# Tangshitao/Semi-supervised-Adaptive-Distillation

Measured on AMD Instinct MI355X. Metric: images/sec (student+teacher fwd + student bwd) R50-FPN distill, 1/2/4/8 MI355X, higher is better.
Workload: dtype f32

## Files before the change

### include/ssad_kernels.h

```cpp
#ifndef SSAD_KERNELS_H_
#define SSAD_KERNELS_H_

#include <stddef.h>
#include <stdint.h>

#ifdef __cplusplus
extern "C" {
#endif

#define SSAD_API __attribute__((visibility("default")))

#define SSAD_E_BADARG (-1)
#define SSAD_E_WORKSPACE (-2)
#define SSAD_MAX_LEVELS 8
#define SSAD_MAX_CONV_PROBLEMS 24
#define SSAD_MAX_POWSUM_INPUTS 8

typedef void* ssad_stream_t;


typedef struct {
  float gamma;
  float alpha;
  float beta;
// ... 176 lines not shown
    const float* bias, int Cout, int Cin, int flags, ssad_stream_t stream);

SSAD_API size_t ssad_conv_split_filter_floats(int M, int K);
SSAD_API int ssad_conv_split_pack_filters(const ssad_pack_entry* entries_host, int n_entries, ssad_stream_t stream);
SSAD_API size_t ssad_conv3x3_split_workspace_bytes(const ssad_conv_level* levels_host, int n_levels, int Cin);
SSAD_API int ssad_conv3x3_forward_split(
    const ssad_conv_level* levels_host, int n_levels, const float* packed,
    const float* bias, int Cout, int Cin, int flags, void* workspace, size_t workspace_bytes,
    const unsigned* amax_in, unsigned* amax_out, ssad_stream_t stream);

SSAD_API size_t ssad_conv3x3_wgrad_workspace_bytes(
    const ssad_conv_level* levels_host, int n_levels, int Cout, int Cin);

SSAD_API int ssad_conv3x3_wgrad(
    const ssad_conv_level* levels_host, int n_levels, float* dW, float* db,
    int Cout, int Cin, int accumulate, void* workspace, size_t workspace_bytes,
    ssad_stream_t stream);

SSAD_API size_t ssad_conv3x3_wgrad_split_workspace_bytes(
    const ssad_conv_level* levels_host, int n_levels, int Cout, int Cin);
SSAD_API int ssad_conv3x3_wgrad_split(
    const ssad_conv_level* levels_host, int n_levels, float* dW, float* db,
    int Cout, int Cin, int accumulate, void* workspace, size_t workspace_bytes,
    ssad_stream_t stream);
SSAD_API int ssad_conv3x3_wgrad_split_amax(
    const ssad_conv_level* levels_host, int n_levels, float* dW, float* db,
    int Cout, int Cin, int accumulate, void* workspace, size_t workspace_bytes,
    const unsigned* x_amax, const unsigned* dy_amax, ssad_stream_t stream);

SSAD_API int ssad_split_absmax_levels(const ssad_conv_level* levels_host, int n, int channels, int field,
                                      unsigned* words, ssad_stream_t stream);
SSAD_API int ssad_split_absmax(const float* x, long long n, unsigned* word, ssad_stream_t stream);


SSAD_API size_t ssad_retinanet_anchor_labels_workspace_bytes(
    int levels, int A, int k_min, const int* field_sizes_host, int N, int Gmax);
SSAD_API int ssad_retinanet_anchor_labels(
    const double* cell_anchors, int levels, int A, int k_min, const int* field_sizes_host,
    const int* crop_h_host, const int* crop_w_host, const float* gt_boxes,
    const int* gt_classes, const int* gt_counts, int N, int Gmax, int num_classes,
    float positive_overlap, float negative_overlap, int* const* labels_out_host,
    float* const* locs_out_host, float* const* targets_out_host, int capacity,
    int* counts_out, float* fg_bg_out, void* workspace, size_t workspace_bytes,
    ssad_stream_t stream);


SSAD_API int ssad_conv_out_size(int in, int kernel, int dilation, int pad_a, int pad_b, int stride);
SSAD_API int ssad_im2col(const float* x, int C, int H, int W, int kh, int kw, int dil_h, int dil_w,
                         int pad_t, int pad_l, int pad_b, int pad_r, int stride_h, int stride_w,
                         float* col, ssad_stream_t stream);
SSAD_API int ssad_im2col_batched(const float* x, int N, int C, int H, int W, int kernel, int stride,
                                 int pad, float* col, ssad_stream_t stream);
SSAD_API int ssad_col2im(const float* col, int C, int H, int W, int kh, int kw, int dil_h,
                         int dil_w, int pad_t, int pad_l, int pad_b, int pad_r, int stride_h,
                         int stride_w, float* x, ssad_stream_t stream);
SSAD_API int ssad_channel_sum(const float* dy, int N, int C, int HW, float* out, int accumulate,
                              ssad_stream_t stream);
SSAD_API int ssad_relu_grad_rowsum(const float* y, const float* dy, float* dx, float* rowsum, int N,
                                   int C, int HW, ssad_stream_t stream);
SSAD_API int ssad_conv1x1_bias_act(const float* x, const float* w, const float* bias,
                                   const float* residual, float* y, int N, int C, int P, int M,
                                   int relu, ssad_stream_t stream);
SSAD_API int ssad_conv1x1_bias_act2(const float* x, int C1, const float* x2, int C2, const float* w,
                                    const float* bias, const float* residual, float* y, int N, int P,
                                    int M, int relu, ssad_stream_t stream);
#define SSAD_GEMM_RELU 1
#define SSAD_GEMM_ACCUMULATE 8
typedef struct ssad_gemm_conv {
  const float* a;
  const float* x;
  float* y;
  const float* bias;
  const float* residual;
  const float* mask;
  int lda, N, K, P, M, flags;
} ssad_gemm_conv;
SSAD_API int ssad_conv1x1_gemm(const ssad_gemm_conv* desc_host, ssad_stream_t stream);
SSAD_API size_t ssad_conv1x1_gemm_split_workspace_bytes(const ssad_gemm_conv* desc_host);
SSAD_API int ssad_conv1x1_gemm_split(const ssad_gemm_conv* desc_host, void* workspace, size_t workspace_bytes,
                                     ssad_stream_t stream);
SSAD_API int ssad_conv1x1_gemm_split_amax(const ssad_gemm_conv* desc_host, const float* packed_a, const unsigned* x_amax,
                                          unsigned* y_amax_out, void* workspace, size_t workspace_bytes,
                                          ssad_stream_t stream);
typedef struct ssad_gemm_pack_entry {
  const float* a;
  float* dst;
  int lda, K, M;
} ssad_gemm_pack_entry;
SSAD_API size_t ssad_gemm_split_filter_floats(int K, int M);
SSAD_API int ssad_gemm_split_pack_filters(const ssad_gemm_pack_entry* entries_host, int n_entries, ssad_stream_t stream);
SSAD_API int ssad_conv_implicit_gemm(const ssad_gemm_conv* d, int C, int H, int W, int kernel, int stride, int pad,
                                     ssad_stream_t stream);
SSAD_API size_t ssad_conv_implicit_gemm_workspace_bytes(int N, int M, int C, int H, int W, int kernel, int stride,
                                                        int pad);
SSAD_API int ssad_conv_implicit_gemm_ws(const ssad_gemm_conv* d, int C, int H, int W, int kernel, int stride, int pad,
                                        void* workspace, size_t workspace_bytes, ssad_stream_t stream);
SSAD_API size_t ssad_conv_kxk_wgrad_workspace_bytes(int N, int C, int H, int W, int M, int kernel, int stride,
                                                    int pad);
SSAD_API int ssad_conv_kxk_wgrad(const float* x, const float* dy, int N, int C, int H, int W, int M, int kernel,
                                 int stride, int pad, float* dw, int accumulate, void* workspace,
                                 size_t workspace_bytes, ssad_stream_t stream);
SSAD_API size_t ssad_conv_kxk_dgrad_workspace_bytes(int N, int C, int H, int W, int M, int kernel, int stride,
                                                    int pad);
SSAD_API int ssad_conv_kxk_dgrad(const float* w, const float* dy, int N, int C, int H, int W, int M, int kernel,
                                 int stride, int pad, float* dx, const float* mask, int accumulate, void* workspace,
                                 size_t workspace_bytes, ssad_stream_t stream);
SSAD_API int ssad_transpose_filter(const float* w, int M, int K, int ldm, float* wt, ssad_stream_t stream);
#define SSAD_MAX_TRANSPOSE_ENTRIES 64
typedef struct ssad_transpose_entry {
  const float* w;
  float* wt;
  int M, K, ldm;
  int reserved;
} ssad_transpose_entry;
SSAD_API int ssad_transpose_filters(const ssad_transpose_entry* entries_host, int n_entries, ssad_stream_t stream);
SSAD_API size_t ssad_conv1x1_wgrad_workspace_bytes(int N, int C, int P, int M);
SSAD_API int ssad_conv1x1_wgrad(const float* x, const float* dy, int N, int C, int P, int M, float* dw,
                                int accumulate, void* workspace, size_t workspace_bytes,
                                ssad_stream_t stream);
SSAD_API size_t ssad_conv1x1_wgrad_split_workspace_bytes(int N, int C, int P, int M);
SSAD_API int ssad_conv1x1_wgrad_split(const float* x, const float* dy, int N, int C, int P, int M, float* dw,
                                      int accumulate, void* workspace, size_t workspace_bytes,
                                      ssad_stream_t stream);
SSAD_API int ssad_conv1x1_wgrad_split_amax(const float* x, const float* dy, int N, int C, int P, int M, float* dw,
                                           int accumulate, void* workspace, size_t workspace_bytes,
                                           const unsigned* x_amax, const unsigned* dy_amax, ssad_stream_t stream);
SSAD_API int ssad_subsample(const float* x, int N, int C, int H, int W, int stride, float* y,
                            ssad_stream_t stream);
SSAD_API int ssad_subsample_grad(const float* dy, int N, int C, int H, int W, int stride, int accumulate,
                                 float* dx, ssad_stream_t stream);
SSAD_API long long ssad_grouped_conv3x3_filter_floats(int C, int group);
SSAD_API int ssad_grouped_conv3x3_pack_filter(const float* w, int C, int group, float* packed,
                                              ssad_stream_t stream);
SSAD_API int ssad_grouped_conv3x3_forward(const float* x, const float* packed, const float* bias, int N, int C,
                                          int H, int W, int group, int stride, int relu, float* y,
                                          ssad_stream_t stream);
SSAD_API int ssad_max_pool_forward(const float* x, int N, int C, int H, int W, int kh, int kw,
                                   int stride_h, int stride_w, int pad_t, int pad_l, int pad_b,
                                   int pad_r, float* y, ssad_stream_t stream);
SSAD_API int ssad_max_pool3x3s2_bias_relu(const float* x, const float* bias, int N, int C, int H,
                                          int W, int relu, float* y, ssad_stream_t stream);
SSAD_API int ssad_max_pool_backward(const float* x, const float* y, const float* dy, int N, int C,
                                    int H, int W, int kh, int kw, int stride_h, int stride_w,
                                    int pad_t, int pad_l, int pad_b, int pad_r, float* dx,
                                    ssad_stream_t stream);

SSAD_API size_t ssad_retinanet_detect_workspace_bytes(
    int levels, int A, int C, const int* H_host, const int* W_host, int pre_nms_topn);
SSAD_API int ssad_retinanet_detect(
    const float* const* cls_prob_host, const float* const* box_pred_host,
    const double* cell_anchors, int levels, int A, int C, int k_min, const int* H_host,
    const int* W_host, float inference_th, int pre_nms_topn, float nms_thresh, int dets_per_im,
    float im_scale, int im_height, int im_width, float bbox_xform_clip, float* dets_out,
    int* count_out, void* workspace, size_t workspace_bytes, ssad_stream_t stream);

SSAD_API int ssad_f16_pack_activations(const float* x_nchw, int N, int C, int H, int W, float scale,
                                       void* x_blocked, ssad_stream_t stream);
SSAD_API int ssad_f16_unpack_activations(const void* x_blocked, int N, int C, int H, int W, float scale,
                                         float* x_nchw, ssad_stream_t stream);
SSAD_API int ssad_f16_pack_activations_dyn(const float* x_nchw, int N, int C, int H, int W, float scale,
                                           const float* scale_dev, void* x_blocked, ssad_stream_t stream);
SSAD_API int ssad_f16_unpack_activations_dyn(const void* x_blocked, int N, int C, int H, int W, float scale,
                                             const float* scale_dev, float* x_nchw, ssad_stream_t stream);
SSAD_API int ssad_f16_block_activations(const void* x_nchw_f16, int N, int C, int H, int W,
                                        void* x_blocked, ssad_stream_t stream);
SSAD_API int ssad_f16_unblock_activations(const void* x_blocked, int N, int C, int H, int W,
// ... 95 lines not shown
```

### semi-supervised-adaptive-distillation_amd/csrc/kernels/gemm_split.hip

```cpp
#include <stdlib.h>

#include <mutex>

#include "split_common.h"

namespace {

using namespace ssad_split;

constexpr int PT = 128;
constexpr int MT = 256;
constexpr int HDR = 16;

__host__ __device__ constexpr int cdiv(int a, int b) { return (a + b - 1) / b; }

__global__ __launch_bounds__(kThreads) void gsplit_pack_a_kernel(const float* __restrict__ a, int lda, int K, int M,
                                                                 const unsigned* __restrict__ amax, float* __restrict__ dst) {
  const int KB = (K + 7) >> 3;
  const long long slots = (long long)KB * M;
  const float s = pow2f(15 - split_exponent(amax[0]));
  if (blockIdx.x == 0 && threadIdx.x < HDR) reinterpret_cast<unsigned*>(dst)[threadIdx.x] = threadIdx.x == 0 ? amax[0] : 0u;
  uint4* out = reinterpret_cast<uint4*>(dst + HDR);
  for (long long i = (long long)blockIdx.x * kThreads + threadIdx.x; i < slots; i += (long long)gridDim.x * kThreads) {
    const int m = (int)(i % M), kb = (int)(i / M);
    float v[8];
#pragma unroll
    for (int j = 0; j < 8; ++j) v[j] = kb * 8 + j < K ? a[(long long)(kb * 8 + j) * lda + m] : 0.0f;
    half8 hi, lo;
    split8(v, s, hi, lo);
    out[i] = __builtin_bit_cast(uint4, hi);
    out[slots + i] = __builtin_bit_cast(uint4, lo);
  }
}

struct GPackTable {
  ssad_gemm_pack_entry e[SSAD_MAX_PACK_ENTRIES];
  int count;
};
__global__ __launch_bounds__(kThreads) void gsplit_zero_kernel(const GPackTable t) {
  for (int i = (int)threadIdx.x; i < t.count * HDR; i += kThreads) reinterpret_cast<unsigned*>(t.e[i / HDR].dst)[i % HDR] = 0u;
}
__global__ __launch_bounds__(kThreads) void gsplit_amax_kernel(const GPackTable t) {
  const ssad_gemm_pack_entry& E = t.e[blockIdx.y];
  unsigned m = 0;
  for (int k = (int)blockIdx.x; k < E.K; k += (int)gridDim.x)
    for (int j = (int)threadIdx.x; j < E.M; j += kThreads) {
      const unsigned a = __float_as_uint(E.a[(long long)k * E.lda + j]) & 0x7fffffffu;
      m = m > a ? m : a;
    }
#pragma unroll
  for (int o = 32; o > 0; o >>= 1) {
    const unsigned other = (unsigned)__shfl_xor((int)m, o, 64);
    m = m > other ? m : other;
  }
  __shared__ unsigned red[kThreads / 64];
  if ((threadIdx.x & 63) == 0) red[threadIdx.x >> 6] = m;
  __syncthreads();
  if (threadIdx.x == 0) {
    for (int w = 1; w < kThreads / 64; ++w) m = m > red[w] ? m : red[w];
    if (m) atomicMax(reinterpret_cast<unsigned*>(E.dst), m);
  }
}
__global__ __launch_bounds__(kThreads) void gsplit_pack_multi_kernel(const GPackTable t) {
  const ssad_gemm_pack_entry& E = t.e[blockIdx.y];
  const int KB = (E.K + 7) >> 3;
  const long long slots = (long long)KB * E.M;
  const float s = pow2f(15 - split_exponent(reinterpret_cast<const unsigned*>(E.dst)[0]));
  uint4* out = reinterpret_cast<uint4*>(E.dst + HDR);
  for (long long i = (long long)blockIdx.x * kThreads + threadIdx.x; i < slots; i += (long long)gridDim.x * kThreads) {
    const int m = (int)(i % E.M), kb = (int)(i / E.M);
    float v[8];
#pragma unroll
    for (int j = 0; j < 8; ++j) v[j] = kb * 8 + j < E.K ? E.a[(long long)(kb * 8 + j) * E.lda + m] : 0.0f;
    half8 hi, lo;
    split8(v, s, hi, lo);
    out[i] = __builtin_bit_cast(uint4, hi);
    out[slots + i] = __builtin_bit_cast(uint4, lo);
  }
}

#ifndef GFLY_ABLATE
#define GFLY_ABLATE 0
#endif
constexpr int FKC = 32;
constexpr int FWG = 512;
constexpr int F_XP = (FKC / 8) * PT * 16;
constexpr int F_WP = (FKC / 8) * MT * 16;
constexpr int F_STAGE = 2 * F_XP + 2 * F_WP;
constexpr int F_LDS = 2 * F_STAGE;

struct FArgs {
  const float* x;
  const float* ap;
  float* y;
  const float* bias;
  const float* residual;
  const float* mask;
  const unsigned* amax;
  unsigned* amax_out;
  int N, K, P, M, relu, accumulate;
  int ptiles, mblocks, items;
};

__global__ __launch_bounds__(FWG, 1) void gemm_fly_kernel(const FArgs q) {
  extern __shared__ __attribute__((aligned(16))) char flds[];
  const int tid = threadIdx.x, lane = tid & 63;
  const int wave = __builtin_amdgcn_readfirstlane(tid >> 6);
  const int wm = wave & 3, wp = wave >> 2;
  const int j = lane & 31, h = lane >> 5;
  const int K = q.K, M = q.M, P = q.P;
  const int KB = (K + 7) >> 3;
  const int nchunks = (K + FKC - 1) / FKC;

  int n, p0, ocb;
  {
    const int it = (int)blockIdx.x;
    const int xcd = it & 7, seq = it >> 3;
    const int mb = seq % q.mblocks;
    const int t = (seq / q.mblocks) * 8 + xcd;
    if (t >= q.N * q.ptiles) return;
    n = t / q.ptiles;
    p0 = (t - n * q.ptiles) * PT;
    ocb = mb * MT;
  }
  const unsigned w_lo_off = (unsigned)((long long)KB * M * 16);
  const __amdgpu_buffer_rsrc_t xrs = uniform_rsrc(q.x, (unsigned)((long long)q.N * K * P * 4));
  const __amdgpu_buffer_rsrc_t wrs = uniform_rsrc(q.ap + HDR, 2u * w_lo_off);
  const float sx = pow2f(15 - split_exponent(q.amax[0]));

  float xv[8];
  f32x4 wv[4];
  const int fpx = tid & (PT - 1), fkg = tid >> 7;
  const int fco = tid & (MT - 1), fkq = tid >> 8;
  const unsigned xbase = p0 + fpx < P ? (unsigned)((((long long)n * K + 8 * fkg) * P + p0 + fpx) * 4) : kOob;
  const int P4 = P * 4;
  auto fetch = [&](int c) {
    const int soff = __builtin_amdgcn_readfirstlane(c * FKC * P4);
#pragma unroll
    for (int e = 0; e < 8; ++e)
      xv[e] = __builtin_bit_cast(float, __builtin_amdgcn_raw_buffer_load_b32(
          xrs, c * FKC + 8 * fkg + e < K ? xbase : kOob, soff + e * P4, 0));
#pragma unroll
    for (int i = 0; i < 2; ++i) {
      const int kb = c * (FKC / 8) + fkq + 2 * i;
      const unsigned vo = (kb < KB && ocb + fco < M) ? (unsigned)((kb * M + ocb + fco) * 16) : kOob;
      wv[2 * i] = __builtin_bit_cast(f32x4, __builtin_amdgcn_raw_buffer_load_b128(wrs, vo, 0, 0));
      wv[2 * i + 1] = __builtin_bit_cast(f32x4, __builtin_amdgcn_raw_buffer_load_b128(wrs, vo, (int)w_lo_off, 0));
    }
  };
  auto put = [&](char* stage) {
    half8 hi, lo;
    split8(xv, sx, hi, lo);
    char* px = stage + (fkg * PT + fpx) * 16;
    *reinterpret_cast<half8*>(px) = hi;
    *reinterpret_cast<half8*>(px + F_XP) = lo;
#pragma unroll
    for (int i = 0; i < 2; ++i) {
      char* pw = stage + 2 * F_XP + ((fkq + 2 * i) * MT + fco) * 16;
      *reinterpret_cast<f32x4*>(pw) = wv[2 * i];
      *reinterpret_cast<f32x4*>(pw + F_WP) = wv[2 * i + 1];
    }
  };

  float16v acc[2][2];
#pragma unroll
  for (int i = 0; i < 2; ++i)
#pragma unroll
    for (int tt = 0; tt < 2; ++tt)
#pragma unroll
      for (int r = 0; r < 16; ++r) acc[i][tt][r] = 0.0f;

  auto step = [&](const char* stage, int st) {
    half8 ah[2], al[2], bh[2], bl[2];
    const int kg = 2 * st + h;
#pragma unroll
    for (int i = 0; i < 2; ++i) {
      const char* pw = stage + 2 * F_XP + (kg * MT + wm * 64 + i * 32 + j) * 16;
      ah[i] = *reinterpret_cast<const half8*>(pw);
      al[i] = *reinterpret_cast<const half8*>(pw + F_WP);
      const char* px = stage + (kg * PT + wp * 64 + i * 32 + j) * 16;
      bh[i] = *reinterpret_cast<const half8*>(px);
      bl[i] = *reinterpret_cast<const half8*>(px + F_XP);
    }
#pragma unroll
    for (int pr = 0; pr < ((GFLY_ABLATE & 8) ? 0 : (GFLY_ABLATE & 4) ? 1 : 3); ++pr)
#pragma unroll
      for (int i = 0; i < 2; ++i)
#pragma unroll
        for (int tt = 0; tt < 2; ++tt)
          acc[i][tt] = __builtin_amdgcn_mfma_f32_32x32x16_f16(pr == 1 ? al[i] : ah[i], pr == 2 ? bl[tt] : bh[tt],
                                                              acc[i][tt], 0, 0, 0);
    if (GFLY_ABLATE & 8) {
#pragma unroll
      for (int i = 0; i < 2; ++i) { acc[i][0][0] += (float)ah[i][0] + (float)al[i][1]; acc[i][1][0] += (float)bh[i][0] + (float)bl[i][1]; }
    }
  };

  fetch(0);
  put(flds);
  fetch(1);
  __syncthreads();
  for (int c = 0; c < nchunks; ++c) {
    const char* stage = flds + (c & 1) * F_STAGE;
    char* other = flds + ((c & 1) ^ 1) * F_STAGE;
    __builtin_amdgcn_sched_barrier(0);
    step(stage, 0);
    if (!(GFLY_ABLATE & 2)) put(other);
    __builtin_amdgcn_sched_barrier(0);
    if (!(GFLY_ABLATE & 1)) fetch(c + 2);
    __builtin_amdgcn_sched_barrier(0);
    step(stage, 1);
    __syncthreads();
  }

  const int oc_w = ocb + wm * 64;
  unsigned pvo[2];
#pragma unroll
  for (int tt = 0; tt < 2; ++tt) {
    const int px = p0 + wp * 64 + 32 * tt + j;
    pvo[tt] = px < P ? (unsigned)((((long long)n * M + 4 * h) * P + px) * 4) : kOob;
  }
  const int e2 = split_exponent(q.amax[0]) + split_exponent(reinterpret_cast<const unsigned*>(q.ap)[0]) - 30;
  const bool one_scale = e2 >= -126 && e2 <= 127;
  const float sc1 = one_scale ? pow2f(e2) : pow2f(split_exponent(q.amax[0]) - 15);
  const float sc2 = one_scale ? 1.0f : pow2f(split_exponent(reinterpret_cast<const unsigned*>(q.ap)[0]) - 15);
  const unsigned ybytes = (unsigned)((long long)q.N * M * P * 4);
  const __amdgpu_buffer_rsrc_t yrs = uniform_rsrc(q.y, ybytes);
  const __amdgpu_buffer_rsrc_t rrs = uniform_rsrc(q.residual ? (const void*)q.residual : (const void*)q.y, q.residual ? ybytes : 0u);
  const __amdgpu_buffer_rsrc_t mrs = uniform_rsrc(q.mask ? (const void*)q.mask : (const void*)q.y, q.mask ? ybytes : 0u);
  const __amdgpu_buffer_rsrc_t brs = uniform_rsrc(q.bias ? (const void*)q.bias : (const void*)q.y, q.bias ? (unsigned)M * 4u : 0u);
  const bool relu = q.relu, has_res = q.residual != nullptr, has_mask = q.mask != nullptr, accum = q.accumulate;
  const bool ragged = (M & 7) != 0;
  unsigned ymax = 0;
#pragma unroll
  for (int i = 0; i < 2; ++i) {
    const int oc0 = oc_w + i * 32;
    float4 bq[4];
#pragma unroll
    for (int g = 0; g < 4; ++g)
      bq[g] = __builtin_bit_cast(float4, __builtin_amdgcn_raw_buffer_load_b128(brs, (unsigned)h * 16u, (oc0 + 8 * g) * 4, 0));
#pragma unroll
    for (int tt = 0; tt < 2; ++tt) {
      float rs[16], mk[16], old[16];
#pragma unroll
      for (int r = 0; r < 16; ++r) {
        const int ch = oc0 + 8 * (r >> 2) + (r & 3);
        const unsigned vo = (ch < M && (!ragged || ch + 4 * h < M)) ? pvo[tt] : kOob;
        rs[r] = has_res ? __builtin_bit_cast(float, __builtin_amdgcn_raw_buffer_load_b32(rrs, vo, ch * P4, 0)) : 0.0f;
        mk[r] = has_mask ? __builtin_bit_cast(float, __builtin_amdgcn_raw_buffer_load_b32(mrs, vo, ch * P4, 0)) : 1.0f;
        old[r] = accum ? __builtin_bit_cast(float, __builtin_amdgcn_raw_buffer_load_b32(yrs, vo, ch * P4, 0)) : 0.0f;
      }
#pragma unroll
      for (int g = 0; g < 4; ++g) {
        if (oc0 + 8 * g >= M) continue;
#pragma unroll
        for (int e = 0; e < 4; ++e) {
          const int r = 4 * g + e;
          float v = one_scale ? fmaf(acc[i][tt][r], sc1, bq[g][e]) : acc[i][tt][r] * sc1 * sc2 + bq[g][e];
          v += rs[r];
          if (relu) v = fmaxf(v, 0.0f);
          if (has_mask) v = mk[r] > 0.0f ? v : 0.0f;
          v += old[r];
          const unsigned vo = (!ragged || oc0 + 8 * g + 4 * h + e < M) ? pvo[tt] : kOob;
          __builtin_amdgcn_raw_buffer_store_b32(__builtin_bit_cast(unsigned, v), yrs, vo, (oc0 + 8 * g + e) * P4, 0);
          const unsigned av = __builtin_bit_cast(unsigned, v) & 0x7fffffffu;
          if (vo != kOob) ymax = ymax > av ? ymax : av;
        }
      }
    }
  }
  if (q.amax_out) {
#pragma unroll
    for (int o = 32; o > 0; o >>= 1) {
      const unsigned other = (unsigned)__shfl_xor((int)ymax, o, 64);
      ymax = ymax > other ? ymax : other;
    }
    __syncthreads();
    unsigned* red = reinterpret_cast<unsigned*>(flds);
    if (lane == 0) red[wave] = ymax;
    __syncthreads();
    if (tid == 0) {
      for (int w = 1; w < FWG / 64; ++w) ymax = ymax > red[w] ? ymax : red[w];
      if (ymax) atomicMax(q.amax_out, ymax);
    }
  }
}

constexpr int WT = 256;
constexpr int WPX = 32;
constexpr int W_PL = (WPX / 8) * WT * 16;
constexpr int W_STAGE = 4 * W_PL;
constexpr int W_LDS = 2 * W_STAGE;

struct WPArgs {
  const float* x;
  const float* dy;
  float* slabs;
  const unsigned* xa;
  const unsigned* da;
  int N, C, P, M;
  int mtiles, ctiles, shares, per_share, total, cpi;
  int xcd_runs;
};

__global__ __launch_bounds__(FWG, 1) void wpoint_split_kernel(const WPArgs q) {
  extern __shared__ __attribute__((aligned(16))) char wlds[];
  const int tid = threadIdx.x, lane = tid & 63;
  const int wave = __builtin_amdgcn_readfirstlane(tid >> 6);
  const int wm = wave & 1, wc = wave >> 1;
  const int j = lane & 31, h = lane >> 5;
  const int P = q.P;

  const int tiles = q.mtiles * q.ctiles;
  int share, tile;
  if (q.xcd_runs) {
    const int xcd = blockIdx.x & 7, jj = blockIdx.x >> 3;
    share = xcd * q.xcd_runs + jj / tiles;
    tile = jj % tiles;
  } else {
    share = blockIdx.x / tiles;
    tile = blockIdx.x % tiles;
  }
  const int m0 = (tile / q.ctiles) * WT, c0 = (tile % q.ctiles) * WT;
  const int q_begin = share * q.per_share;
  const int q_end = q_begin + q.per_share < q.total ? q_begin + q.per_share : q.total;

  const __amdgpu_buffer_rsrc_t xrs = uniform_rsrc(q.x, (unsigned)((long long)q.N * q.C * P * 4));
  const __amdgpu_buffer_rsrc_t drs = uniform_rsrc(q.dy, (unsigned)((long long)q.N * q.M * P * 4));
  const float sx = pow2f(15 - split_exponent(q.xa[0]));
  const float sd = pow2f(15 - split_exponent(q.da[0]));

  float dv[2][8], xv[2][8];
  const int fpg = tid & 3, fch = tid >> 2;
  auto fetch = [&](int ck) {
    const int n = __builtin_amdgcn_readfirstlane(ck / q.cpi);
    const int p = (ck - n * q.cpi) * WPX + 8 * fpg;
    const bool pok = ck < q.total && p < P;
#pragma unroll
    for (int i = 0; i < 2; ++i) {
      const int m = m0 + fch + 128 * i, c = c0 + fch + 128 * i;
      const unsigned od = (pok && m < q.M) ? (unsigned)((((long long)n * q.M + m) * P + p) * 4) : kOob;
      const unsigned ox = (pok && c < q.C) ? (unsigned)((((long long)n * q.C + c) * P + p) * 4) : kOob;
      const f32x4 d0 = __builtin_bit_cast(f32x4, __builtin_amdgcn_raw_buffer_load_b128(drs, od, 0, 0));
      const f32x4 d1 = __builtin_bit_cast(f32x4, __builtin_amdgcn_raw_buffer_load_b128(drs, od, 16, 0));
      const f32x4 x0 = __builtin_bit_cast(f32x4, __builtin_amdgcn_raw_buffer_load_b128(xrs, ox, 0, 0));
      const f32x4 x1 = __builtin_bit_cast(f32x4, __builtin_amdgcn_raw_buffer_load_b128(xrs, ox, 16, 0));
#pragma unroll
      for (int e = 0; e < 4; ++e) { dv[i][e] = d0[e]; dv[i][4 + e] = d1[e]; xv[i][e] = x0[e]; xv[i][4 + e] = x1[e]; }
    }
  };
  auto put = [&](char* stage) {
#pragma unroll
    for (int i = 0; i < 2; ++i) {
      half8 hi, lo;
      char* pd = stage + (fpg * WT + fch + 128 * i) * 16;
      split8(dv[i], sd, hi, lo);
      *reinterpret_cast<half8*>(pd) = hi;
      *reinterpret_cast<half8*>(pd + W_PL) = lo;
      split8(xv[i], sx, hi, lo);
      *reinterpret_cast<half8*>(pd + 2 * W_PL) = hi;
      *reinterpret_cast<half8*>(pd + 3 * W_PL) = lo;
    }
  };

  float16v acc[4][2];
// ... 20 lines not shown
      for (int i = 0; i < 2; ++i) {
        const char* pd = stage + (kg * WT + wm * 128 + (2 * ip + i) * 32 + j) * 16;
        ah[i] = *reinterpret_cast<const half8*>(pd);
        al[i] = *reinterpret_cast<const half8*>(pd + W_PL);
      }
#pragma unroll
      for (int pr = 0; pr < 3; ++pr)
#pragma unroll
        for (int i = 0; i < 2; ++i)
#pragma unroll
          for (int tt = 0; tt < 2; ++tt)
            acc[2 * ip + i][tt] = __builtin_amdgcn_mfma_f32_32x32x16_f16(pr == 1 ? al[i] : ah[i], pr == 2 ? bl[tt] : bh[tt],
                                                                         acc[2 * ip + i][tt], 0, 0, 0);
    }
  };

  if (q_begin < q_end) {
    fetch(q_begin);
    put(wlds);
    fetch(q_begin + 1 < q_end ? q_begin + 1 : q.total);
  }
  __syncthreads();
  for (int ck = q_begin; ck < q_end; ++ck) {
    const char* stage = wlds + ((ck - q_begin) & 1) * W_STAGE;
    char* other = wlds + (((ck - q_begin) & 1) ^ 1) * W_STAGE;
    __builtin_amdgcn_sched_barrier(0);
    step(stage, 0);
    put(other);
    __builtin_amdgcn_sched_barrier(0);
    fetch(ck + 2 < q_end ? ck + 2 : q.total);
    __builtin_amdgcn_sched_barrier(0);
    step(stage, 1);
    __syncthreads();
  }

  const int Mp = q.mtiles * WT, Cp = q.ctiles * WT;
  float* slab = q.slabs + (long long)share * Mp * Cp;
#pragma unroll
  for (int i = 0; i < 4; ++i)
#pragma unroll
    for (int tt = 0; tt < 2; ++tt)
#pragma unroll
      for (int r = 0; r < 16; ++r) {
        const int m = m0 + wm * 128 + i * 32 + 8 * (r >> 2) + 4 * h + (r & 3);
        const int c = c0 + wc * 64 + tt * 32 + j;
        slab[(long long)m * Cp + c] = acc[i][tt][r];
      }
}

__global__ __launch_bounds__(256) void wpoint_reduce_kernel(const float* __restrict__ slabs, int shares, int Mp, int Cp,
                                                            int M, int C, const unsigned* __restrict__ xa,
                                                            const unsigned* __restrict__ da,
                                                            float* __restrict__ dw, int accumulate) {
  const long long e = (long long)blockIdx.x * 256 + threadIdx.x;
  if (e >= (long long)M * C) return;
  const int m = (int)(e / C), c = (int)(e - (long long)m * C);
  const float* p = slabs + (long long)m * Cp + c;
  const long long stride = (long long)Mp * Cp;
  float s = 0.0f;
  for (int sh = 0; sh < shares; ++sh) s += p[sh * stride];
  s = (s * pow2f(split_exponent(xa[0]) - 15)) * pow2f(split_exponent(da[0]) - 15);
  dw[e] = accumulate ? dw[e] + s : s;
}

int wpoint_plan(int N, int C, int P, int M, WPArgs* a) {
  if (N <= 0 || C <= 0 || P <= 0 || M <= 0 || (P & 7)) return SSAD_E_BADARG;
  if ((long long)N * C * P * 4 >= (1LL << 31) || (long long)N * M * P * 4 >= (1LL << 31)) return SSAD_E_BADARG;
  a->N = N; a->C = C; a->P = P; a->M = M;
  a->mtiles = cdiv(M, WT); a->ctiles = cdiv(C, WT);
  a->cpi = cdiv(P, WPX);
  a->total = N * a->cpi;
  const int cus = ssad_cu_count(), tiles = a->mtiles * a->ctiles;
  int s = cus / tiles;
  if (s < 1) s = 1;
  if (s >= 8) s &= ~7;
  while (s > 1 && a->total / s < 4) --s;
  a->per_share = cdiv(a->total, s);
  a->shares = cdiv(a->total, a->per_share);
  a->xcd_runs = (a->shares % 8 == 0) ? a->shares / 8 : 0;
  return 0;
}

struct GPlan {
  size_t amax_off, a_off, total;
};
int make_plan(const ssad_gemm_conv* d, GPlan* p) {
  if (!d || d->N <= 0 || d->K <= 0 || d->P <= 0 || d->M <= 0 || d->lda < d->M) return SSAD_E_BADARG;
  const int KB = (d->K + 7) >> 3;
  const long long aslots = (long long)KB * d->M;
  if ((long long)d->N * d->K * d->P * 4 >= (1LL << 31) || (long long)d->N * d->M * d->P * 4 >= (1LL << 31) ||
      aslots * 32 >= (1LL << 31))
    return SSAD_E_BADARG;
  p->amax_off = 0;
  p->a_off = 256;
  p->total = p->a_off + (size_t)HDR * 4 + (size_t)aslots * 32;
  return 0;
}

}

extern "C" {

size_t ssad_conv1x1_gemm_split_workspace_bytes(const ssad_gemm_conv* d) {
  GPlan p;
  return make_plan(d, &p) ? 0 : p.total;
}

size_t ssad_gemm_split_filter_floats(int K, int M) {
  if (K <= 0 || M <= 0) return 0;
  return (size_t)HDR + (size_t)((K + 7) >> 3) * M * 8;
}

int ssad_gemm_split_pack_filters(const ssad_gemm_pack_entry* entries_host, int n_entries, ssad_stream_t stream_) {
  hipStream_t stream = (hipStream_t)stream_;
  if (!entries_host || n_entries < 0) return SSAD_E_BADARG;
  for (int base = 0; base < n_entries; base += SSAD_MAX_PACK_ENTRIES) {
    GPackTable t;
    const int cnt = n_entries - base < SSAD_MAX_PACK_ENTRIES ? n_entries - base : SSAD_MAX_PACK_ENTRIES;
    long long most = 0;
    for (int i = 0; i < cnt; ++i) {
      t.e[i] = entries_host[base + i];
      if (!t.e[i].a || !t.e[i].dst || t.e[i].K <= 0 || t.e[i].M <= 0 || t.e[i].lda < t.e[i].M) return SSAD_E_BADARG;
      const long long slots = (long long)((t.e[i].K + 7) >> 3) * t.e[i].M;
      if (slots > most) most = slots;
    }
    t.count = cnt;
    hipLaunchKernelGGL(gsplit_zero_kernel, dim3(1), dim3(kThreads), 0, stream, t);
    hipLaunchKernelGGL(gsplit_amax_kernel, dim3(64u, (unsigned)cnt), dim3(kThreads), 0, stream, t);
    long long bx = (most + kThreads - 1) / kThreads;
    if (bx > 256) bx = 256;
    hipLaunchKernelGGL(gsplit_pack_multi_kernel, dim3((unsigned)bx, (unsigned)cnt), dim3(kThreads), 0, stream, t);
  }
  return (int)hipGetLastError();
}

int ssad_conv1x1_gemm_split(const ssad_gemm_conv* d, void* workspace, size_t workspace_bytes, ssad_stream_t stream_) {
  return ssad_conv1x1_gemm_split_amax(d, nullptr, nullptr, nullptr, workspace, workspace_bytes, stream_);
}

int ssad_conv1x1_gemm_split_amax(const ssad_gemm_conv* d, const float* packed_a, const unsigned* x_amax,
                                 unsigned* y_amax_out, void* workspace, size_t workspace_bytes, ssad_stream_t stream_) {
  hipStream_t stream = (hipStream_t)stream_;
  GPlan p;
  const int rc = make_plan(d, &p);
  if (rc) return rc;
  if (!d->a || !d->x || !d->y) return SSAD_E_BADARG;
  if ((d->flags & SSAD_GEMM_ACCUMULATE) && (d->bias || d->residual)) return SSAD_E_BADARG;
  if (!workspace || workspace_bytes < p.total) return SSAD_E_WORKSPACE;
  char* ws = (char*)workspace;
  unsigned* amax = (unsigned*)(ws + p.amax_off);
  float* apk = (float*)(ws + p.a_off);
  const int KB = (d->K + 7) >> 3;
  AmaxTable at;
  for (int l = 0; l < kMaxLv; ++l) { at.x[l] = nullptr; at.n[l] = 0; at.block_start[l] = 0; }
  at.count = 2;
  at.amax = amax;
  at.x[0] = d->x; at.n[0] = (long long)d->N * d->K * d->P;
  at.x[1] = d->a; at.n[1] = (long long)d->K * d->lda;
  int blocks = 0;
  for (int l = 0; l < 2; ++l) {
    at.block_start[l] = blocks;
    long long nb = (at.n[l] / 4 + kThreads * 32 - 1) / (kThreads * 32);
    blocks += (int)(nb < 1 ? 1 : nb > 512 ? 512 : nb);
  }
  for (int l = 2; l <= kMaxLv; ++l) at.block_start[l] = blocks;
  if (x_amax && packed_a) {
  } else {
    if (x_amax) { at.n[0] = 0; }
    if (packed_a) { at.n[1] = 0; }
    (void)hipMemsetAsync(amax, 0, 256, stream);
    hipLaunchKernelGGL(split_absmax_kernel, dim3((unsigned)blocks), dim3(kThreads), 0, stream, at);
    if (!packed_a) {
      long long bx = ((long long)KB * d->M + kThreads - 1) / kThreads;
      if (bx > 1024) bx = 1024;
      hipLaunchKernelGGL(gsplit_pack_a_kernel, dim3((unsigned)bx), dim3(kThreads), 0, stream, d->a, d->lda, d->K, d->M,
                         (const unsigned*)(amax + 1), apk);
    }
  }
  FArgs f;
  f.x = d->x; f.ap = packed_a ? packed_a : apk; f.y = d->y; f.bias = d->bias; f.residual = d->residual; f.mask = d->mask;
  f.amax = x_amax ? x_amax : amax;
  f.amax_out = y_amax_out;
  f.N = d->N; f.K = d->K; f.P = d->P; f.M = d->M;
  f.relu = (d->flags & SSAD_GEMM_RELU) ? 1 : 0;
  f.accumulate = (d->flags & SSAD_GEMM_ACCUMULATE) ? 1 : 0;
  f.ptiles = cdiv(d->P, PT);
  f.mblocks = cdiv(d->M, MT);
  const long long tiles = (long long)d->N * f.ptiles;
  if (tiles * f.mblocks >= (1LL << 30)) return SSAD_E_BADARG;
  f.items = (int)(cdiv((int)tiles, 8) * 8 * f.mblocks);
  static std::once_flag lds_once;
  std::call_once(lds_once, [&] {
    (void)hipFuncSetAttribute((const void*)gemm_fly_kernel, hipFuncAttributeMaxDynamicSharedMemorySize, F_LDS);
  });
  hipLaunchKernelGGL(gemm_fly_kernel, dim3((unsigned)f.items), dim3(FWG), F_LDS, stream, f);
  return (int)hipGetLastError();
}

int ssad_split_absmax(const float* x, long long n, unsigned* word, ssad_stream_t stream_) {
  if (!x || !word || n <= 0) return SSAD_E_BADARG;
  AmaxTable at;
  for (int l = 0; l < kMaxLv; ++l) { at.x[l] = nullptr; at.n[l] = 0; at.block_start[l] = 0; }
  at.count = 1;
  at.amax = word;
  at.x[0] = x; at.n[0] = n;
  long long nb = (n / 4 + kThreads * 32 - 1) / (kThreads * 32);
  const int blocks = (int)(nb < 1 ? 1 : nb > 512 ? 512 : nb);
  for (int l = 1; l <= kMaxLv; ++l) at.block_start[l] = blocks;
  hipLaunchKernelGGL(split_absmax_kernel, dim3((unsigned)blocks), dim3(kThreads), 0, (hipStream_t)stream_, at);
  return (int)hipGetLastError();
}

size_t ssad_conv1x1_wgrad_split_workspace_bytes(int N, int C, int P, int M) {
  WPArgs a;
  if (wpoint_plan(N, C, P, M, &a)) return 0;
  return 256 + sizeof(float) * (size_t)a.shares * a.mtiles * WT * a.ctiles * WT;
}

int ssad_conv1x1_wgrad_split(const float* x, const float* dy, int N, int C, int P, int M, float* dw, int accumulate,
                             void* workspace, size_t workspace_bytes, ssad_stream_t stream_) {
  return ssad_conv1x1_wgrad_split_amax(x, dy, N, C, P, M, dw, accumulate, workspace, workspace_bytes, nullptr, nullptr,
                                       stream_);
}

int ssad_conv1x1_wgrad_split_amax(const float* x, const float* dy, int N, int C, int P, int M, float* dw, int accumulate,
                                  void* workspace, size_t workspace_bytes, const unsigned* x_amax,
                                  const unsigned* dy_amax, ssad_stream_t stream_) {
  hipStream_t stream = (hipStream_t)stream_;
  if ((x_amax == nullptr) != (dy_amax == nullptr)) return SSAD_E_BADARG;
  WPArgs a;
  const int rc = wpoint_plan(N, C, P, M, &a);
  if (rc) return rc;
  if (!x || !dy || !dw) return SSAD_E_BADARG;
  const size_t need = 256 + sizeof(float) * (size_t)a.shares * a.mtiles * WT * a.ctiles * WT;
  if (!workspace || workspace_bytes < need) return SSAD_E_WORKSPACE;
  unsigned* amax = (unsigned*)workspace;
  a.x = x; a.dy = dy;
  a.xa = x_amax ? x_amax : amax;
  a.da = dy_amax ? dy_amax : amax + 1;
  a.slabs = (float*)((char*)workspace + 256);
  if (!x_amax) {
  AmaxTable at;
  for (int l = 0; l < kMaxLv; ++l) { at.x[l] = nullptr; at.n[l] = 0; at.block_start[l] = 0; }
  at.count = 2;
  at.amax = amax;
  at.x[0] = x; at.n[0] = (long long)N * C * P;
  at.x[1] = dy; at.n[1] = (long long)N * M * P;
  int blocks = 0;
  for (int l = 0; l < 2; ++l) {
    at.block_start[l] = blocks;
    long long nb = (at.n[l] / 4 + kThreads * 32 - 1) / (kThreads * 32);
    blocks += (int)(nb < 1 ? 1 : nb > 512 ? 512 : nb);
  }
  for (int l = 2; l <= kMaxLv; ++l) at.block_start[l] = blocks;
  (void)hipMemsetAsync(amax, 0, 256, stream);
  hipLaunchKernelGGL(split_absmax_kernel, dim3((unsigned)blocks), dim3(kThreads), 0, stream, at);
  }
  static std::once_flag lds_once;
  std::call_once(lds_once, [&] {
    (void)hipFuncSetAttribute((const void*)wpoint_split_kernel, hipFuncAttributeMaxDynamicSharedMemorySize, W_LDS);
  });
  hipLaunchKernelGGL(wpoint_split_kernel, dim3((unsigned)(a.mtiles * a.ctiles * a.shares)), dim3(FWG), W_LDS, stream, a);
  const long long n = (long long)M * C;
  hipLaunchKernelGGL(wpoint_reduce_kernel, dim3((unsigned)((n + 255) / 256)), dim3(256), 0, stream,
                     (const float*)a.slabs, a.shares, a.mtiles * WT, a.ctiles * WT, M, C, a.xa, a.da, dw, accumulate);
  return (int)hipGetLastError();
}

}
```

Measured before the change: 230.1.

## Add stream-K split of K chunks for small-grid split-fp16 1x1 GEMM

When the tile count is small relative to the CU count, the 1x1 conv GEMM now spreads K-chunk units evenly across workgroups (stream-K). Partial accumulators go to workspace slots, and the last contributor, detected through a tagged atomic counter, reduces them and runs the epilogue. The non-stream-K kernel also preloads both LDS operand sets before issuing MFMAs, and strided-lda filters get their own amax pass. The aim is to fill idle CUs on small late-stage GEMMs, at the cost of extra workspace traffic and cross-workgroup synchronisation.

```diff
diff --git a/include/ssad_kernels.h b/include/ssad_kernels.h
--- a/include/ssad_kernels.h
+++ b/include/ssad_kernels.h
@@ -282,6 +282,7 @@
 SSAD_API int ssad_conv1x1_gemm_split_amax(const ssad_gemm_conv* desc_host, const float* packed_a, const unsigned* x_amax,
                                           unsigned* y_amax_out, void* workspace, size_t workspace_bytes,
                                           ssad_stream_t stream);
+SSAD_API int ssad_conv1x1_gemm_split_plan(const ssad_gemm_conv* desc_host, int* out);
 typedef struct ssad_gemm_pack_entry {
   const float* a;
   float* dst;
diff --git a/semi-supervised-adaptive-distillation_amd/csrc/kernels/gemm_split.hip b/semi-supervised-adaptive-distillation_amd/csrc/kernels/gemm_split.hip
--- a/semi-supervised-adaptive-distillation_amd/csrc/kernels/gemm_split.hip
+++ b/semi-supervised-adaptive-distillation_amd/csrc/kernels/gemm_split.hip
@@ -87,7 +87,10 @@
 constexpr int F_XP = (FKC / 8) * PT * 16;
 constexpr int F_WP = (FKC / 8) * MT * 16;
 constexpr int F_STAGE = 2 * F_XP + 2 * F_WP;
-constexpr int F_LDS = 2 * F_STAGE;
+constexpr int F_LDS = 2 * F_STAGE + 64;
+constexpr int F_SLOT = MT * PT * 4;
+typedef unsigned u32x4 __attribute__((vector_size(16)));
+constexpr unsigned long long F_TAG = 0x7f8a5e1d6d2b0000ull;
 
 struct FArgs {
   const float* x;
@@ -98,11 +101,23 @@
   const float* mask;
   const unsigned* amax;
   unsigned* amax_out;
+  unsigned long long* cnt;
+  float* slots;
   int N, K, P, M, relu, accumulate;
-  int ptiles, mblocks, items;
+  int ptiles, mblocks, items, nch, units, wgs, xcd_major;
 };
 
-__global__ __launch_bounds__(FWG, 1) void gemm_fly_kernel(const FArgs q) {
+__host__ __device__ inline int fly_begin(int L, int units, int wgs) { return (int)((long long)L * units / wgs); }
+__host__ __device__ inline int fly_owner(int u, int units, int wgs) { return (int)(((long long)(u + 1) * wgs - 1) / units); }
+__host__ __device__ inline int fly_slot(int L, int i, int nch, int units, int wgs) {
+  return 2 * L + (fly_begin(L, units, wgs) / nch == i ? 0 : 1);
+}
+
+template <bool STREAMK>
+__global__ void gemm_fly_kernel(const FArgs q);
+
+template <>
+__global__ __launch_bounds__(FWG, 1) void gemm_fly_kernel<false>(const FArgs q) {
   extern __shared__ __attribute__((aligned(16))) char flds[];
   const int tid = threadIdx.x, lane = tid & 63;
   const int wave = __builtin_amdgcn_readfirstlane(tid >> 6);
@@ -170,18 +185,21 @@
 #pragma unroll
       for (int r = 0; r < 16; ++r) acc[i][tt][r] = 0.0f;
 
-  auto step = [&](const char* stage, int st) {
-    half8 ah[2], al[2], bh[2], bl[2];
+  struct Ops { half8 ah[2], al[2], bh[2], bl[2]; };
+  auto load = [&](const char* stage, int st, Ops& o) {
     const int kg = 2 * st + h;
 #pragma unroll
     for (int i = 0; i < 2; ++i) {
       const char* pw = stage + 2 * F_XP + (kg * MT + wm * 64 + i * 32 + j) * 16;
-      ah[i] = *reinterpret_cast<const half8*>(pw);
-      al[i] = *reinterpret_cast<const half8*>(pw + F_WP);
+      o.ah[i] = *reinterpret_cast<const half8*>(pw);
+      o.al[i] = *reinterpret_cast<const half8*>(pw + F_WP);
       const char* px = stage + (kg * PT + wp * 64 + i * 32 + j) * 16;
-      bh[i] = *reinterpret_cast<const half8*>(px);
-      bl[i] = *reinterpret_cast<const half8*>(px + F_XP);
-    }
+      o.bh[i] = *reinterpret_cast<const half8*>(px);
+      o.bl[i] = *reinterpret_cast<const half8*>(px + F_XP);
+    }
+  };
+  auto step = [&](const Ops& o) {
+    const half8 (&ah)[2] = o.ah, (&al)[2] = o.al, (&bh)[2] = o.bh, (&bl)[2] = o.bl;
 #pragma unroll
     for (int pr = 0; pr < ((GFLY_ABLATE & 8) ? 0 : (GFLY_ABLATE & 4) ? 1 : 3); ++pr)
 #pragma unroll
@@ -203,13 +221,16 @@
   for (int c = 0; c < nchunks; ++c) {
     const char* stage = flds + (c & 1) * F_STAGE;
     char* other = flds + ((c & 1) ^ 1) * F_STAGE;
+    Ops o0, o1;
     __builtin_amdgcn_sched_barrier(0);
-    step(stage, 0);
+    load(stage, 0, o0);
+    load(stage, 1, o1);
+    step(o0);
     if (!(GFLY_ABLATE & 2)) put(other);
     __builtin_amdgcn_sched_barrier(0);
     if (!(GFLY_ABLATE & 1)) fetch(c + 2);
     __builtin_amdgcn_sched_barrier(0);
-    step(stage, 1);
+    step(o1);
     __syncthreads();
   }
 
@@ -281,6 +302,271 @@
     __syncthreads();
     if (tid == 0) {
       for (int w = 1; w < FWG / 64; ++w) ymax = ymax > red[w] ? ymax : red[w];
+      if (ymax) atomicMax(q.amax_out, ymax);
+    }
+  }
+}
+
+template <>
+__global__ __launch_bounds__(FWG, 1) void gemm_fly_kernel<true>(const FArgs q) {
+  extern __shared__ __attribute__((aligned(16))) char flds[];
+  unsigned* red = reinterpret_cast<unsigned*>(flds + 2 * F_STAGE);
+  const int tid = threadIdx.x, lane = tid & 63;
+  const int wave = __builtin_amdgcn_readfirstlane(tid >> 6);
+  const int wm = wave & 3, wp = wave >> 2;
+  const int j = lane & 31, h = lane >> 5;
+  const int K = q.K, M = q.M, P = q.P;
+  const int KB = (K + 7) >> 3;
+  const int nch = q.nch, units = q.units, wgs = q.wgs;
+
+  const int b = __builtin_amdgcn_readfirstlane((int)blockIdx.x);
+  const int L = q.xcd_major ? (b & 7) * (wgs >> 3) + (b >> 3) : b;
+  const int u0 = fly_begin(L, units, wgs), u1 = fly_begin(L + 1, units, wgs);
+  if (u0 >= u1) return;
+
+  const unsigned w_lo_off = (unsigned)((long long)KB * M * 16);
+  const __amdgpu_buffer_rsrc_t xrs = uniform_rsrc(q.x, (unsigned)((long long)q.N * K * P * 4));
+  const __amdgpu_buffer_rsrc_t wrs = uniform_rsrc(q.ap + HDR, 2u * w_lo_off);
+  const float sx = pow2f(15 - split_exponent(q.amax[0]));
+
+  float xv[8];
+  f32x4 wv[4];
+  const int fpx = tid & (PT - 1), fkg = tid >> 7;
+  const int fco = tid & (MT - 1), fkq = tid >> 8;
+  const int P4 = P * 4;
+  int fg = u0, fi = u0 / nch, fc = u0 - fi * nch;
+  unsigned f_xbase = 0;
+  int f_ocb = 0;
+  auto locate = [&]() {
+    const int t = fi / q.mblocks;
+    f_ocb = (fi - t * q.mblocks) * MT;
+    const int n = t / q.ptiles, p0 = (t - n * q.ptiles) * PT;
+    f_xbase = p0 + fpx < P ? (unsigned)((((long long)n * K + 8 * fkg) * P + p0 + fpx) * 4) : kOob;
+  };
+  locate();
+  auto fetch = [&]() {
+    const int soff = __builtin_amdgcn_readfirstlane(fc * FKC * P4);
+#pragma unroll
+    for (int e = 0; e < 8; ++e)
+      xv[e] = __builtin_bit_cast(float, __builtin_amdgcn_raw_buffer_load_b32(
+          xrs, fc * FKC + 8 * fkg + e < K ? f_xbase : kOob, soff + e * P4, 0));
+#pragma unroll
+    for (int i = 0; i < 2; ++i) {
+      const int kb = fc * (FKC / 8) + fkq + 2 * i;
+      const unsigned vo = (kb < KB && f_ocb + fco < M) ? (unsigned)((kb * M + f_ocb + fco) * 16) : kOob;
+      wv[2 * i] = __builtin_bit_cast(f32x4, __builtin_amdgcn_raw_buffer_load_b128(wrs, vo, 0, 0));
+      wv[2 * i + 1] = __builtin_bit_cast(f32x4, __builtin_amdgcn_raw_buffer_load_b128(wrs, vo, (int)w_lo_off, 0));
+    }
+    ++fg;
+    if (++fc == nch) {
+      fc = 0;
+      ++fi;
+      if (fg < u1) locate();
+    }
+    if (fg >= u1) {
+      f_xbase = kOob;
+      f_ocb = M;
+    }
+  };
+  auto put = [&](char* stage) {
+    half8 hi, lo;
+    split8(xv, sx, hi, lo);
+    char* px = stage + (fkg * PT + fpx) * 16;
+    *reinterpret_cast<half8*>(px) = hi;
+    *reinterpret_cast<half8*>(px + F_XP) = lo;
+#pragma unroll
+    for (int i = 0; i < 2; ++i) {
+      char* pw = stage + 2 * F_XP + ((fkq + 2 * i) * MT + fco) * 16;
+      *reinterpret_cast<f32x4*>(pw) = wv[2 * i];
+      *reinterpret_cast<f32x4*>(pw + F_WP) = wv[2 * i + 1];
+    }
+  };
+
+  float16v acc[2][2];
+  auto zero_acc = [&]() {
+#pragma unroll
+    for (int i = 0; i < 2; ++i)
+#pragma unroll
+      for (int tt = 0; tt < 2; ++tt)
+#pragma unroll
+        for (int r = 0; r < 16; ++r) acc[i][tt][r] = 0.0f;
+  };
+  zero_acc();
+
+  auto step = [&](const char* stage, int st) {
+    half8 ah[2], al[2], bh[2], bl[2];
+    const int kg = 2 * st + h;
+#pragma unroll
+    for (int i = 0; i < 2; ++i) {
+      const char* pw = stage + 2 * F_XP + (kg * MT + wm * 64 + i * 32 + j) * 16;
+      ah[i] = *reinterpret_cast<const half8*>(pw);
+      al[i] = *reinterpret_cast<const half8*>(pw + F_WP);
+      const char* px = stage + (kg * PT + wp * 64 + i * 32 + j) * 16;
+      bh[i] = *reinterpret_cast<const half8*>(px);
+      bl[i] = *reinterpret_cast<const half8*>(px + F_XP);
+    }
+#pragma unroll
+    for (int pr = 0; pr < ((GFLY_ABLATE & 8) ? 0 : (GFLY_ABLATE & 4) ? 1 : 3); ++pr)
+#pragma unroll
+      for (int i = 0; i < 2; ++i)
+#pragma unroll
+        for (int tt = 0; tt < 2; ++tt)
+          acc[i][tt] = __builtin_amdgcn_mfma_f32_32x32x16_f16(pr == 1 ? al[i] : ah[i], pr == 2 ? bl[tt] : bh[tt],
+                                                              acc[i][tt], 0, 0, 0);
+    if (GFLY_ABLATE & 8) {
+#pragma unroll
+      for (int i = 0; i < 2; ++i) { acc[i][0][0] += (float)ah[i][0] + (float)al[i][1]; acc[i][1][0] += (float)bh[i][0] + (float)bl[i][1]; }
+    }
+  };
+
+  const int e2 = split_exponent(q.amax[0]) + split_exponent(reinterpret_cast<const unsigned*>(q.ap)[0]) - 30;
+  const bool one_scale = e2 >= -126 && e2 <= 127;
+  const float sc1 = one_scale ? pow2f(e2) : pow2f(split_exponent(q.amax[0]) - 15);
+  const float sc2 = one_scale ? 1.0f : pow2f(split_exponent(reinterpret_cast<const unsigned*>(q.ap)[0]) - 15);
+  const unsigned ybytes = (unsigned)((long long)q.N * M * P * 4);
+  const __amdgpu_buffer_rsrc_t yrs = uniform_rsrc(q.y, ybytes);
+  const __amdgpu_buffer_rsrc_t rrs = uniform_rsrc(q.residual ? (const void*)q.residual : (const void*)q.y, q.residual ? ybytes : 0u);
+  const __amdgpu_buffer_rsrc_t mrs = uniform_rsrc(q.mask ? (const void*)q.mask : (const void*)q.y, q.mask ? ybytes : 0u);
+  const __amdgpu_buffer_rsrc_t brs = uniform_rsrc(q.bias ? (const void*)q.bias : (const void*)q.y, q.bias ? (unsigned)M * 4u : 0u);
+  const __amdgpu_buffer_rsrc_t srs = uniform_rsrc(q.slots, (unsigned)(2 * wgs) * (unsigned)F_SLOT);
+  const bool relu = q.relu, has_res = q.residual != nullptr, has_mask = q.mask != nullptr, accum = q.accumulate;
+  const bool ragged = (M & 7) != 0;
+  unsigned ymax = 0;
+
+  auto epilogue = [&](int item) {
+    const int t = item / q.mblocks;
+    const int ocb = (item - t * q.mblocks) * MT;
+    const int n = t / q.ptiles, p0 = (t - n * q.ptiles) * PT;
+    const int oc_w = ocb + wm * 64;
+    unsigned pvo[2];
+#pragma unroll
+    for (int tt = 0; tt < 2; ++tt) {
+      const int px = p0 + wp * 64 + 32 * tt + j;
+      pvo[tt] = px < P ? (unsigned)((((long long)n * M + 4 * h) * P + px) * 4) : kOob;
+    }
+#pragma unroll
+    for (int i = 0; i < 2; ++i) {
+      const int oc0 = oc_w + i * 32;
+      float4 bq[4];
+#pragma unroll
+      for (int g = 0; g < 4; ++g)
+        bq[g] = __builtin_bit_cast(float4, __builtin_amdgcn_raw_buffer_load_b128(brs, (unsigned)h * 16u, (oc0 + 8 * g) * 4, 0));
+#pragma unroll
+      for (int tt = 0; tt < 2; ++tt) {
+        float rs[16], mk[16], old[16];
+#pragma unroll
+        for (int r = 0; r < 16; ++r) {
+          const int ch = oc0 + 8 * (r >> 2) + (r & 3);
+          const unsigned vo = (ch < M && (!ragged || ch + 4 * h < M)) ? pvo[tt] : kOob;
+          rs[r] = has_res ? __builtin_bit_cast(float, __builtin_amdgcn_raw_buffer_load_b32(rrs, vo, ch * P4, 0)) : 0.0f;
+          mk[r] = has_mask ? __builtin_bit_cast(float, __builtin_amdgcn_raw_buffer_load_b32(mrs, vo, ch * P4, 0)) : 1.0f;
+          old[r] = accum ? __builtin_bit_cast(float, __builtin_amdgcn_raw_buffer_load_b32(yrs, vo, ch * P4, 0)) : 0.0f;
+        }
+#pragma unroll
+        for (int g = 0; g < 4; ++g) {
+          if (oc0 + 8 * g >= M) continue;
+#pragma unroll
+          for (int e = 0; e < 4; ++e) {
+            const int r = 4 * g + e;
+            float v = one_scale ? fmaf(acc[i][tt][r], sc1, bq[g][e]) : acc[i][tt][r] * sc1 * sc2 + bq[g][e];
+            v += rs[r];
+            if (relu) v = fmaxf(v, 0.0f);
+            if (has_mask) v = mk[r] > 0.0f ? v : 0.0f;
+            v += old[r];
+            const unsigned vo = (!ragged || oc0 + 8 * g + 4 * h + e < M) ? pvo[tt] : kOob;
+            __builtin_amdgcn_raw_buffer_store_b32(__builtin_bit_cast(unsigned, v), yrs, vo, (oc0 + 8 * g + e) * P4, 0);
+            const unsigned av = __builtin_bit_cast(unsigned, v) & 0x7fffffffu;
+            if (vo != kOob) ymax = ymax > av ? ymax : av;
+          }
+        }
+      }
+    }
+  };
+
+  auto combine = [&](int item) -> bool {
+    const int first = fly_owner(item * nch, units, wgs), parts = fly_owner(item * nch + nch - 1, units, wgs) - first + 1;
+    const unsigned mine = (unsigned)fly_slot(L, item, nch, units, wgs) * (unsigned)F_SLOT;
+#pragma unroll
+    for (int v = 0; v < 16; ++v) {
+      const float16v& a = acc[v >> 3][(v >> 2) & 1];
+      const int r = 4 * (v & 3);
+      const f32x4 o = {a[r], a[r + 1], a[r + 2], a[r + 3]};
+      __builtin_amdgcn_raw_buffer_store_b128(__builtin_bit_cast(u32x4, o), srs, mine + (unsigned)(v * FWG + tid) * 16u, 0,
+                                             16 );
+    }
+    asm volatile("s_waitcnt vmcnt(0)" ::: "memory");
+    __syncthreads();
+    if (tid == 0) {
+      typedef __attribute__((address_space(1))) unsigned long long gu64;
+      gu64* w = (gu64*)(q.cnt + first);
+      unsigned long long old = __hip_atomic_load(w, __ATOMIC_RELAXED, __HIP_MEMORY_SCOPE_AGENT), nw;
+      for (;;) {
+        nw = ((old & ~0xffffull) == F_TAG ? old : F_TAG) + 1;
+        if (__hip_atomic_compare_exchange_strong(w, &old, nw, __ATOMIC_RELAXED, __ATOMIC_RELAXED, __HIP_MEMORY_SCOPE_AGENT))
+          break;
+      }
+      const bool last = (int)(nw & 0xffffull) == parts;
+      if (last) {
+        __hip_atomic_store(w, 0ull, __ATOMIC_RELAXED, __HIP_MEMORY_SCOPE_AGENT);
+        __builtin_amdgcn_fence(__ATOMIC_ACQUIRE, "agent");
+        asm volatile("s_waitcnt vmcnt(0)" ::: "memory");
+      }
+      red[0] = last ? 1u : 0u;
+    }
+    __syncthreads();
+    if (!red[0]) return false;
+    for (int pt = 0; pt < parts; ++pt) {
+      const unsigned so = (unsigned)fly_slot(first + pt, item, nch, units, wgs) * (unsigned)F_SLOT;
+#pragma unroll
+      for (int v = 0; v < 16; ++v) {
+        float16v& a = acc[v >> 3][(v >> 2) & 1];
+        const int r = 4 * (v & 3);
+        const f32x4 o = __builtin_bit_cast(f32x4, __builtin_amdgcn_raw_buffer_load_b128(srs, so + (unsigned)(v * FWG + tid) * 16u, 0, 0));
+#pragma unroll
+        for (int e = 0; e < 4; ++e) a[r + e] = pt == 0 ? o[e] : a[r + e] + o[e];
+      }
+    }
+    return true;
+  };
+
+  int item = u0 / nch, c = u0 - item * nch;
+  bool whole = c == 0;
+  fetch();
+  put(flds);
+  fetch();
+  __syncthreads();
+  for (int g = u0; g < u1; ++g) {
+    const char* stage = flds + ((g - u0) & 1) * F_STAGE;
+    char* other = flds + (((g - u0) & 1) ^ 1) * F_STAGE;
+    __builtin_amdgcn_sched_barrier(0);
+    step(stage, 0);
+    if (!(GFLY_ABLATE & 2)) put(other);
+    __builtin_amdgcn_sched_barrier(0);
+    if (!(GFLY_ABLATE & 1)) fetch();
+    __builtin_amdgcn_sched_barrier(0);
+    step(stage, 1);
+    if (c == nch - 1 || g == u1 - 1) {
+      if ((whole && c == nch - 1) || combine(item)) epilogue(item);
+      zero_acc();
+      ++item;
+      c = 0;
+      whole = true;
+    } else {
+      ++c;
+    }
+    __syncthreads();
+  }
+
+  if (q.amax_out) {
+#pragma unroll
+    for (int o = 32; o > 0; o >>= 1) {
+      const unsigned other = (unsigned)__shfl_xor((int)ymax, o, 64);
+      ymax = ymax > other ? ymax : other;
+    }
+    if (lane == 0) red[1 + wave] = ymax;
+    __syncthreads();
+    if (tid == 0) {
+      for (int w = 1; w < FWG / 64; ++w) ymax = ymax > red[1 + w] ? ymax : red[1 + w];
       if (ymax) atomicMax(q.amax_out, ymax);
     }
   }
@@ -467,7 +753,8 @@
 }
 
 struct GPlan {
-  size_t amax_off, a_off, total;
+  size_t amax_off, a_off, cnt_off, slot_off, total;
+  int ptiles, mblocks, items, nch, units, wgs, grid, streamk;
 };
 int make_plan(const ssad_gemm_conv* d, GPlan* p) {
   if (!d || d->N <= 0 || d->K <= 0 || d->P <= 0 || d->M <= 0 || d->lda < d->M) return SSAD_E_BADARG;
@@ -476,9 +763,33 @@
   if ((long long)d->N * d->K * d->P * 4 >= (1LL << 31) || (long long)d->N * d->M * d->P * 4 >= (1LL << 31) ||
       aslots * 32 >= (1LL << 31))
     return SSAD_E_BADARG;
+  p->ptiles = cdiv(d->P, PT);
+  p->mblocks = cdiv(d->M, MT);
+  p->nch = cdiv(d->K, FKC);
+  const long long items = (long long)d->N * p->ptiles * p->mblocks, units = items * p->nch;
+  if (units >= (1LL << 30)) return SSAD_E_BADARG;
+  p->items = (int)items;
+  p->units = (int)units;
+  const int cus = ssad_cu_count();
+  p->streamk = 2 * items <= cus;
+  if (p->streamk) {
+    const int least = p->nch < 4 ? p->nch : 4;
+    long long g = cus;
+    if (g > units / least) g = units / least;
+    if (g >= 8) g &= ~7LL;
+    p->wgs = g < 1 ? 1 : (int)g;
+    p->grid = p->wgs;
+  } else {
+    p->wgs = p->items;
+    p->grid = cdiv(d->N * p->ptiles, 8) * 8 * p->mblocks;
+  }
+  const int slots = p->streamk ? p->wgs : 0;
+  if (2LL * slots * F_SLOT >= (1LL << 31)) return SSAD_E_BADARG;
   p->amax_off = 0;
   p->a_off = 256;
-  p->total = p->a_off + (size_t)HDR * 4 + (size_t)aslots * 32;
+  p->cnt_off = (p->a_off + (size_t)HDR * 4 + (size_t)aslots * 32 + 255) & ~(size_t)255;
+  p->slot_off = (p->cnt_off + (size_t)slots * 8 + 255) & ~(size_t)255;
+  p->total = p->slot_off + (size_t)2 * slots * F_SLOT;
   return 0;
 }
 
@@ -541,7 +852,7 @@
   at.count = 2;
   at.amax = amax;
   at.x[0] = d->x; at.n[0] = (long long)d->N * d->K * d->P;
-  at.x[1] = d->a; at.n[1] = (long long)d->K * d->lda;
+  at.x[1] = d->a; at.n[1] = d->lda == d->M ? (long long)d->K * d->M : 0;
   int blocks = 0;
   for (int l = 0; l < 2; ++l) {
     at.block_start[l] = blocks;
@@ -556,6 +867,12 @@
     (void)hipMemsetAsync(amax, 0, 256, stream);
     hipLaunchKernelGGL(split_absmax_kernel, dim3((unsigned)blocks), dim3(kThreads), 0, stream, at);
     if (!packed_a) {
+      if (d->lda != d->M) {
+        GPackTable t;
+        t.e[0].a = d->a; t.e[0].lda = d->lda; t.e[0].K = d->K; t.e[0].M = d->M; t.e[0].dst = (float*)(amax + 1);
+        t.count = 1;
+        hipLaunchKernelGGL(gsplit_amax_kernel, dim3(64u, 1u), dim3(kThreads), 0, stream, t);
+      }
       long long bx = ((long long)KB * d->M + kThreads - 1) / kThreads;
       if (bx > 1024) bx = 1024;
       hipLaunchKernelGGL(gsplit_pack_a_kernel, dim3((unsigned)bx), dim3(kThreads), 0, stream, d->a, d->lda, d->K, d->M,
@@ -566,20 +883,39 @@
   f.x = d->x; f.ap = packed_a ? packed_a : apk; f.y = d->y; f.bias = d->bias; f.residual = d->residual; f.mask = d->mask;
   f.amax = x_amax ? x_amax : amax;
   f.amax_out = y_amax_out;
+  f.cnt = (unsigned long long*)(ws + p.cnt_off);
+  f.slots = (float*)(ws + p.slot_off);
   f.N = d->N; f.K = d->K; f.P = d->P; f.M = d->M;
   f.relu = (d->flags & SSAD_GEMM_RELU) ? 1 : 0;
   f.accumulate = (d->flags & SSAD_GEMM_ACCUMULATE) ? 1 : 0;
-  f.ptiles = cdiv(d->P, PT);
-  f.mblocks = cdiv(d->M, MT);
-  const long long tiles = (long long)d->N * f.ptiles;
-  if (tiles * f.mblocks >= (1LL << 30)) return SSAD_E_BADARG;
-  f.items = (int)(cdiv((int)tiles, 8) * 8 * f.mblocks);
+  f.ptiles = p.ptiles; f.mblocks = p.mblocks; f.items = p.items; f.nch = p.nch; f.units = p.units; f.wgs = p.wgs;
+  f.xcd_major = (p.wgs % 8 == 0) ? 1 : 0;
   static std::once_flag lds_once;
   std::call_once(lds_once, [&] {
-    (void)hipFuncSetAttribute((const void*)gemm_fly_kernel, hipFuncAttributeMaxDynamicSharedMemorySize, F_LDS);
+    (void)hipFuncSetAttribute((const void*)gemm_fly_kernel<false>, hipFuncAttributeMaxDynamicSharedMemorySize, F_LDS);
+    (void)hipFuncSetAttribute((const void*)gemm_fly_kernel<true>, hipFuncAttributeMaxDynamicSharedMemorySize, F_LDS);
   });
-  hipLaunchKernelGGL(gemm_fly_kernel, dim3((unsigned)f.items), dim3(FWG), F_LDS, stream, f);
+  if (p.streamk)
+    hipLaunchKernelGGL(gemm_fly_kernel<true>, dim3((unsigned)p.grid), dim3(FWG), F_LDS, stream, f);
+  else
+    hipLaunchKernelGGL(gemm_fly_kernel<false>, dim3((unsigned)p.grid), dim3(FWG), F_LDS, stream, f);
   return (int)hipGetLastError();
+}
+
+int ssad_conv1x1_gemm_split_plan(const ssad_gemm_conv* d, int* out) {
+  GPlan p;
+  const int rc = make_plan(d, &p);
+  if (rc) return rc;
+  if (!out) return SSAD_E_BADARG;
+  int whole = 0, cut = 0, most = 1;
+  for (int i = 0; i < p.items; ++i) {
+    const int parts = fly_owner(i * p.nch + p.nch - 1, p.units, p.wgs) - fly_owner(i * p.nch, p.units, p.wgs) + 1;
+    if (parts == 1) ++whole; else ++cut;
+    if (parts > most) most = parts;
+  }
+  out[0] = p.wgs; out[1] = p.items; out[2] = p.nch; out[3] = p.units;
+  out[4] = whole; out[5] = cut; out[6] = most; out[7] = (int)(p.total >> 20);
+  return 0;
 }
 
 int ssad_split_absmax(const float* x, long long n, unsigned* word, ssad_stream_t stream_) {
```

Result: no change. 231.1 (median of 6 runs) (+0.4%).
